# alphacep/vosk-tts

Hardware: AMD Instinct MI355X
Metric: audio_samples_per_sec (higher is better)
Workload: dtype f32

## Files before the change

vosk_tts_amd/csrc/engine_stages.hip.h:

```cpp
#pragma once
struct PendingLN { const float* raw = nullptr; const float* g = nullptr; const float* b = nullptr; const float* stat = nullptr; int nmb = 0; };

static bool enc_fold_ok(vits_session* s, const EncoderW& E, int B, int T) {
  if (E.layers.empty() || !s->xb || !s->y1b) return false;
  const EncLayerW& L = E.layers[0];
  return conv_takes_ln_prologue(conv_params(L.qkv, s->x, s->qkv, B, T, 1, 0)) &&
         conv_takes_ln_prologue(conv_params(L.f1, s->x, s->ffh, B, T, 1, (E.K - 1) / 2));
}

static void run_encoder(vits_session* s, const EncoderW& E, float* x, const int* len, int B, int T, int cond_layer,
                        int cond_off, const float* final_base, float* final_out, PendingLN* pend = nullptr) {
  vits_model* m = s->m;
  const int H = E.H, K = E.K;
  const int n = (int)E.layers.size();
  const bool fold = enc_fold_ok(s, E, B, T);
  bool pstat = fold && g_ln_stats && s->lnst && H % 16 == 0 && H / 16 <= 16;
  if (pstat) {
    const EncLayerW& L0 = E.layers[0];
    ConvParams Pp = conv_params(L0.f2, s->ffh, s->y1, B, T, 1, (K - 1) / 2);
    Pp.in_mask = 1; Pp.out_mask = 1; Pp.len = len;
    pstat = conv_writes_ln_stats(conv_params(L0.o, s->att, s->y1, B, T, 1, 0)) && conv_writes_ln_stats(Pp);
  }
  PendingLN prev;
  for (int i = 0; i < n; ++i) {
// ... 287 lines not shown
    ConvParams P;
    if (mono) {
      const MonoW& Mo = m->mono[f];
      const bool post_res = hp.flow_type == 5;
      hipLaunchKernelGGL(mono_x0_kernel, dim3(cdiv(Ty, 256), half, B), dim3(256), 0, s->stream, u, s->x, s->fh, s->len_y, I, half, Ty,
                         post_res ? 0.5f : 1.0f);
      run_encoder(s, Mo.enc, s->x, s->len_y, B, Ty, -1, -1, post_res ? nullptr : s->fh, s->fskip);
      {
        ProfScope ps(s, "flow.mono_couple", 2.0 * B * half * half * Ty, "mono_couple_kernel");
        launch_mono_couple_on(s->stream, s->fskip, u, Mo.post_w, Mo.post_b, s->len_y, v, B, half, Ty, post_res ? 1 : 0);
      }
      float* t = u; u = v; v = t;
    }
    if (hp.flow_type == 1) {
      hipLaunchKernelGGL(flow_x0_kernel, dim3(cdiv(Ty, 256), half, B), dim3(256), 0, s->stream, u, s->x, s->fh, s->len_y, I, half, Ty);
      run_encoder(s, C.enc, s->x, s->len_y, B, Ty, -1, -1, s->fh, s->fskip);
      P = conv_params(C.pre, s->fskip, s->fx, B, Ty, 1, 0);
      P.out_mask = 1; P.len = s->len_y;
      mark_masked(s, P, s->len_y);
      launch_conv(s, P, EPI_STORE, "flow.pre");
    } else {
      P = conv_params(C.pre, u, hp.flow_type == 0 ? s->fh : s->fx, B, Ty, 1, 0);
      P.x_ch_off = I - 1; P.x_ch_sign = -1; P.x_bstride = (long long)I * Ty;
      P.out_mask = 1; P.len = s->len_y;
      mark_masked(s, P, s->len_y);
      if (hp.flow_type == 0) P.g[0].y2 = s->x;
      launch_conv(s, P, EPI_STORE, "flow.pre");
      if (hp.flow_type == 0) run_encoder(s, C.enc, s->x, s->len_y, B, Ty, -1, -1, s->fh, s->fx);
    }
    const bool fold = g_wn_fold && !C.rsx.empty() && C.skip_post.w;
    const long long acts_b = (long long)(fold ? L : 1) * H * Ty;
    for (int i = 0; i < L; ++i) {
      float* acts = s->facts + (fold ? (size_t)i * H * Ty : 0);
      P = conv_params(C.in_layers[i], s->fx, acts, B, Ty, 1, (K5 - 1) / 2);
      P.Cout = H; P.H = H; P.y_bstride = acts_b;
      if (m->use_g) { P.bias_b = s->condv; P.bias_b_stride = m->cond_rows; P.bias_b_off = C.cond_off + i * 2 * H; }
      P.in_mask = 1; P.len = s->len_y;
      mark_masked(s, P, s->len_y);
      launch_conv(s, P, EPI_GATE, "flow.wn_in");
      if (fold) {
        if (i == L - 1) break;
        P = conv_params(C.rsx[i], acts, s->fx, B, Ty, 1, 0);
        P.x_bstride = acts_b;
        P.g[0].res = s->fx; P.out_mask = 1; P.len = s->len_y;
        mark_masked(s, P, s->len_y);
        launch_conv(s, P, EPI_STORE, "flow.wn_rs");
        continue;
      }
      P = conv_params(C.rs_layers[i], s->facts, nullptr, B, Ty, 1, 0);
      P.io = s->fx; P.skip = s->fskip; P.H = H; P.first = i == 0; P.last = i == L - 1; P.len = s->len_y;
      P.y_bstride = (long long)H * Ty;
      mark_masked(s, P, s->len_y);
      launch_conv(s, P, EPI_RESSKIP, "flow.wn_rs");
    }
    P = fold ? conv_params(C.skip_post, s->facts, nullptr, B, Ty, 1, 0) : conv_params(C.post, s->fskip, nullptr, B, Ty, 1, 0);
    P.u = u; P.io = v; P.H = half; P.len = s->len_y; P.y_bstride = (long long)I * Ty;
    mark_masked(s, P, s->len_y);
    launch_conv(s, P, EPI_COUPLE, "flow.post");
    float* t = u; u = v; v = t;
  }
  return u;
}

#define VITS_RAGGED_HALO 32
static void set_rag(ConvParams& P, const int* rag, int in_mul, int in_add, int out_mul, int out_add) {
  P.rag = rag; P.rag_in_mul = in_mul; P.rag_in_add = in_add; P.rag_out_mul = out_mul; P.rag_out_add = out_add; P.rag_out_cap_add = 0; P.rag_tab_add = 0;
}
static ConvParams dec_sum_conv(const ConvW& W, const float* const in[3], float in_scale, float slope, float* y, int B, int Cin, int Cout,
                               int Tin, int Tout, int pad_l, int taps, const UpW* U = nullptr, bool reflect = false) {
  ConvParams P = conv_params(W, in[0], y, B, Tin, 1, pad_l);
  P.g[0].x2 = in[1]; P.g[0].x3 = in[2]; P.g[0].K = taps;
  P.Cin = Cin; P.x_bstride = (long long)Cin * Tin;
  P.Cout = Cout; P.Tout = Tout; P.Tout_stride = U ? Tout * U->u : Tout; P.y_bstride = (long long)(U ? U->cout : Cout) * P.Tout_stride;
  P.in_slope = slope; P.in_scale = in_scale; P.reflect = reflect;
  if (U) {
    P.ups_u = U->u; P.ups_cout = U->cout;
    for (int r = 0; r < U->u; ++r) P.ups_shift[r] = U->shift[r];
  }
  return P;
}
static void run_decoder(vits_session* s, const float* z, bool mask_in, int B, int Ty, float* d_audio, long long audio_bstride,
                        bool ragged = false, bool cont = true) {
  vits_model* m = s->m;
  const vits_hparams& hp = m->hp;
  const DecGeom& G = m->geom;
  vits_session::DecBufs& W = s->dec;
  static const DecNeeds alone;
  const DecNeeds& ND = cont ? G.needs : alone;
  const int* rag = nullptr;
  const int* rag_tail = nullptr;
  if (ragged && (B > 1 || s->rag_b1)) {
    hipLaunchKernelGGL(ragged_len_kernel, dim3(cdiv(B + 1, 64)), dim3(64), 0, s->stream, s->len_y, s->len_rag, s->len_tail, B, Ty,
                       0, G.final_rate, ND.tail_cols);
    rag = s->len_rag;
    rag_tail = s->len_tail;
  }
  ConvParams P = conv_params(m->conv_pre, z, W.pre, B, Ty, 1, 3);
  if (mask_in) { P.in_mask = 1; P.len = s->len_y; }
  if (m->cond_dec_off >= 0) { P.bias_b = s->condv; P.bias_b_stride = m->cond_rows; P.bias_b_off = m->cond_dec_off; }
  set_rag(P, rag, 1, 0, 1, ND.pre_out);
  launch_conv(s, P, EPI_STORE, "dec.conv_pre");
  int prod_add = ND.pre_out;
  const float* in[3] = {W.pre, nullptr, nullptr};
  float in_scale = 1.f;
  const int nk = hp.n_resk;
  auto group = [](ConvGroup& g, const ConvW& w, const float* x, float* y, const float* res, int K, int dil) {
    g.x = x; g.w = w.w; g.wb = w.wb; g.bias = w.bias; g.y = y; g.res = res;
    g.K = K; g.dil = dil; g.pad_l = (K - 1) * dil / 2; g.n_sg = w.n_sg;
  };
  for (int i = 0; i < G.n_ups; ++i) {
    const DecGeom::Stage& S = G.st[i];
    const UpW& U = m->ups[i];
    const int p = i & 1, Ti = Ty * S.rate_in, T = Ty * S.rate_out;
    float* y = W.ups[p];
    float* const* xt = W.xt[p];
    float* const* x = W.x[p];
    P = dec_sum_conv(U.w, in, in_scale, 0.1f, y, B, S.cin, U.w.M, Ti, Ti, U.pad_l, U.taps, &U);
    set_rag(P, rag, S.rate_in, prod_add, S.rate_in, ND.ups_q[i]);
    launch_conv(s, P, EPI_STORE, "dec.ups", U.halo);
    prod_add = ND.ups_q[i] * S.u;
    for (int d = 0; d < hp.n_resd; ++d) {
      const ResBlockW* R = &m->rb[(size_t)i * nk];
      P = conv_params(R[0].c1[d], nullptr, nullptr, B, T, 1, 0);
      P.n_groups = nk; P.in_slope = 0.1f;
      for (int j = 0; j < nk; ++j) group(P.g[j], R[j].c1[d], d == 0 ? y : x[j], xt[j], nullptr, R[j].K, R[j].dil[d]);
      set_rag(P, rag, S.rate_out, prod_add, S.rate_out, ND.c1_out[i][d]);
      P.rag_tab_add = ND.c1_out[i][0];
      launch_conv(s, P, EPI_STORE, "dec.res_c1");
      for (int j = 0; j < nk; ++j) group(P.g[j], R[j].c2[d], xt[j], x[j], d == 0 ? y : x[j], R[j].K, 1);
      set_rag(P, rag, S.rate_out, ND.c1_out[i][d], S.rate_out, ND.c2_out[i][d]);
      P.rag_tab_add = ND.c1_out[i][0];
      launch_conv(s, P, EPI_STORE, "dec.res_c2");
      prod_add = ND.c2_out[i][d];
    }
    in[0] = x[0]; in[1] = nk > 1 ? x[1] : nullptr; in[2] = nk > 2 ? x[2] : nullptr;
    in_scale = 1.0f / (float)nk;
  }
  const int T = Ty * G.final_rate, Tp = T + G.reflect, C = G.st[G.n_ups - 1].cout;
  float* post = W.post;
  P = dec_sum_conv(m->conv_post, in, in_scale, 0.01f, post, B, C, G.post_rows, T, Tp, G.post_pad, 7, nullptr, G.reflect);
  set_rag(P, rag, G.final_rate, prod_add, G.final_rate, cont ? ND.post_out : (int)G.reflect);
  P.rag_out_cap_add = G.reflect;
  launch_conv(s, P, EPI_STORE, "dec.conv_post");
  if (!G.reflect) {
    hipLaunchKernelGGL(tanh_copy_kernel, dim3(cdiv(T, 256), B), dim3(256), 0, s->stream, post, d_audio, T, (long long)T, audio_bstride, rag_tail, 1);
    return;
  }
  float* mb = W.mb;
  const int S = hp.subbands, N = hp.istft_n_fft, hop = hp.istft_hop, Tm = T * hop;
  if (!G.has_mb) {
    if (g_tail_impl == 0) {
      ProfScope ps(s, "istft", 0, "istft_tail_kernel<false>");
      TailParams tp{post, m->istft_basis, nullptr, nullptr, d_audio, 1, N, hop, Tp, Tm, 0, audio_bstride, rag_tail, hop};
      hipLaunchKernelGGL(istft_tail_kernel<false>, dim3(cdiv(Tm, TAIL_SB), B), dim3(256), m->tail_lds, s->stream, tp);
    } else {
      ProfScope ps(s, "istft", 0, "istft_kernel");
      hipLaunchKernelGGL(istft_kernel, dim3(cdiv(Tm, 256), 1, B), dim3(256), 0, s->stream, post, m->istft_basis, d_audio, 1, N, hop, Tp, Tm,
                         audio_bstride, rag_tail, hop, 1);
    }
  } else if (g_tail_impl == 0) {
    ProfScope ps(s, "istft_pqmf", 0, "istft_tail_kernel<true>");
    TailParams tp{post, m->istft_basis, m->pqmf, mb, d_audio, S, N, hop, Tp, Tm, hp.pqmf_taps, audio_bstride, rag_tail, hop};
    hipLaunchKernelGGL(istft_tail_kernel<true>, dim3(cdiv(Tm, TAIL_MB), B), dim3(256), m->tail_lds, s->stream, tp);
  } else {
    {
      ProfScope ps(s, "istft", 0, "istft_kernel");
      hipLaunchKernelGGL(istft_kernel, dim3(cdiv(Tm, 256), S, B), dim3(256), 0, s->stream, post, m->istft_basis, mb, S, N, hop, Tp, Tm,
                         (long long)S * Tm, rag_tail, hop, 0);
    }
    {
      ProfScope ps(s, "pqmf", 0, "pqmf_synthesis_kernel");
      hipLaunchKernelGGL(pqmf_synthesis_kernel, dim3(cdiv(Tm * S, 256), B), dim3(256), 0, s->stream, mb, m->pqmf, d_audio, S,
                         hp.pqmf_taps, Tm, audio_bstride, rag_tail, hop * S);
    }
  }
}

struct HostStage {
  vits_model* m; vits_session* s = nullptr; std::vector<void*> tmp;
  PersistScope pscope;
  explicit HostStage(vits_model* m_) : m(m_), pscope(m_ ? m_->device : -1) {}
  ~HostStage() {
    if (s) {
      hipStreamSynchronize(s->stream);
      if (!tmp.empty()) {
        size_t want = s->stage_used + (s->stage_used >> 2) + (1 << 20);
        if (s->stage) hipFree(s->stage);
        s->stage = nullptr; s->stage_bytes = 0;
        void* p = nullptr;
        if (hipMalloc(&p, want) == hipSuccess) { s->stage = static_cast<char*>(p); s->stage_bytes = want; }
      }
      s->stage_used = 0;
      pool_release(m, s);
    }
    for (void* p : tmp) hipFree(p);
  }
  void* raw_alloc(size_t bytes) {
    bytes = align_up(bytes ? bytes : 1, 256);
    const size_t off = s->stage_used;
    s->stage_used += bytes;
    if (off + bytes <= s->stage_bytes) return s->stage + off;
    void* d = nullptr;
    if (hipMalloc(&d, bytes) != hipSuccess) return nullptr;
    tmp.push_back(d);
    return d;
  }
  template <typename T> T* to_dev(const T* h, size_t n) {
    if (!h) return nullptr;
    void* d = raw_alloc(n * sizeof(T));
    if (!d) return nullptr;
    hipMemcpyAsync(d, h, n * sizeof(T), hipMemcpyHostToDevice, s->stream);
    return static_cast<T*>(d);
  }
  template <typename T> T* dev_alloc(size_t n) { return static_cast<T*>(raw_alloc(n * sizeof(T))); }
};

static int begin_stage(HostStage& hs, int B, int Tx, int Ty, int roles = 7) {
  hipError_t e = hipSetDevice(hs.m->device);
  if (e != hipSuccess) return fail(VITS_ERR_DEVICE, "hipSetDevice failed: %s", hipGetErrorString(e));
  TRY(pool_acquire(hs.m, &hs.s));
  hs.s->ps_roles = roles;
  TRY(session_reserve(hs.s, B, Tx, Ty));
  return VITS_OK;
}

static void set_lengths(vits_session* s, const int64_t* d_len64, int* d_len32, int B, int clamp) {
  hipLaunchKernelGGL(lengths_to_i32_kernel, dim3(cdiv(B, 64)), dim3(64), 0, s->stream, d_len64, d_len32, B, clamp);
}


static void forward_device(vits_session* s, const int64_t* d_ids, const int64_t* d_len, int B, int Tx, const float* scales,
                           const int64_t* d_sid, const int32_t* d_forced, int Ty, uint64_t seed, float* d_audio, int64_t cap) {
  s->ragged = B > 1;
  s->tile_keys.clear();
  run_cond(s, d_sid, B, d_len, s->len_x, Tx);
  const bool with_sdp = !d_forced || s->sdp_always;
  float* z;
  if (persist_mask() == (PERSIST_SDP | PERSIST_ENC | PERSIST_FLOW) && B == 1 && Tx == s->Tx && Ty == s->Ty && s->ps_full[with_sdp].ok) {
    persist_launch(s, s->ps_full[with_sdp], "acoustic.persist", nullptr, scales[2], seed, d_ids, d_forced, scales[1], scales[0]);
    s->ea_pending = false;
    z = s->zB;
  } else {
    run_text_encoder(s, d_ids, B, Tx);
    if (with_sdp) run_duration(s, s->x, nullptr, scales[2], seed, B, Tx, true);
    run_durations(s, d_forced, scales[1], B, Tx, Ty);
    run_expand(s, nullptr, Ty, scales[0], seed, s->zA, B, Tx, Ty);
    z = run_flow(s, B, Ty);
  }
  run_decoder(s, z, true, B, Ty, d_audio, cap, true);
  s->ragged = false;
}
```

vosk_tts_amd/csrc/kernels_misc.hip.h:

```cpp
#pragma once
#include <hip/hip_runtime.h>
#include <stdint.h>

#define PI_F 3.14159265358979323846f

__host__ __device__ inline void philox4x32_10(uint32_t c[4], uint32_t k0, uint32_t k1) {
  for (int r = 0; r < 10; ++r) {
    uint64_t p0 = (uint64_t)0xD2511F53u * c[0], p1 = (uint64_t)0xCD9E8D57u * c[2];
    uint32_t n0 = (uint32_t)(p1 >> 32) ^ c[1] ^ k0, n1 = (uint32_t)p1;
    uint32_t n2 = (uint32_t)(p0 >> 32) ^ c[3] ^ k1, n3 = (uint32_t)p0;
    c[0] = n0; c[1] = n1; c[2] = n2; c[3] = n3;
    k0 += 0x9E3779B9u; k1 += 0xBB67AE85u;
  }
}
__device__ inline float philox_normal(uint64_t seed, uint32_t stream, uint32_t row, uint32_t t) {
  uint32_t c[4] = {t, row, stream, 0};
  philox4x32_10(c, (uint32_t)seed, (uint32_t)(seed >> 32));
  float u1 = ((float)c[0] + 0.5f) * (1.0f / 4294967296.0f);
  float u2 = ((float)c[1] + 0.5f) * (1.0f / 4294967296.0f);
  if (u1 < 1e-12f) u1 = 1e-12f;
  return sqrtf(-2.0f * logf(u1)) * cosf(6.28318530717958647692f * u2);
}

struct SynthDev {
// ... 771 lines not shown
    int d = 0;
    if (t < L) {
      if (forced) d = forced[(long long)b * T + t];
      else {
        const float lw = ea_z ? (ea_z[((long long)b * 2 + ea_row) * T + t] - ea_mu) * ea_sc : logw[(long long)b * T + t];
        d = (int)ceilf(expf(lw) * length_scale);
      }
    }
    if (d < 0) d = 0;
    dur[(long long)b * T + t] = d;
    s += d;
  }
  part[tid] = s;
  __syncthreads();
  if (tid == 0) {
    int run = 0;
    for (int i = 0; i < 256; ++i) { int v = part[i]; part[i] = run; run += v; }
    int yl = run < 1 ? 1 : run;
    if (Tcap > 0 && yl > Tcap) { atomicOr(err, 4); yl = Tcap; }
    ylen32[b] = yl;
    if (ylen64) ylen64[b] = yl;
  }
  __syncthreads();
  int run = part[tid];
  for (int t = t0; t < t0 + per && t < T; ++t) {
    run += dur[(long long)b * T + t];
    cum[(long long)b * T + t] = run;
  }
}

#define EXPAND_CPB 16
__global__ void __launch_bounds__(256) expand_prior_kernel(const float* stats, const int* cum, const int* ylen, const float* noise,
                                                           long long noise_stride, float noise_scale, uint64_t seed, float* z_p,
                                                           int I, int Tx, int Ty, int solo, const SynthDev* dv,
                                                           const unsigned long long* item_seeds) {
  const int f = blockIdx.x * 64 + (threadIdx.x & 63), cl = threadIdx.x >> 6, b = blockIdx.z;
  if (f >= Ty) return;
  if (dv) { noise_scale = dv->scales[0]; seed = dv->seed; }
  const int* cb = cum + (long long)b * Tx;
  int tok = -1;
  if (f < ylen[b] && f < cb[Tx - 1]) {
    int lo = 0, hi = Tx - 1;
    while (lo < hi) { int mid = (lo + hi) >> 1; if (cb[mid] > f) hi = mid; else lo = mid + 1; }
    tok = lo;
  }
  const int tk = tok >= 0 ? tok : 0;
#pragma unroll
  for (int i = 0; i < EXPAND_CPB / 4; ++i) {
    const int c = blockIdx.y * EXPAND_CPB + i * 4 + cl;
    if (c >= I) break;
    const float mu_ = stats[((long long)b * 2 * I + c) * Tx + tk];
    const float ls_ = stats[((long long)b * 2 * I + I + c) * Tx + tk];
    const float mu = tok >= 0 ? mu_ : 0.f, ls = tok >= 0 ? ls_ : 0.f;
    const float e = noise ? noise[((long long)b * I + c) * noise_stride + f]
                          : (solo ? philox_normal(item_seeds ? item_seeds[b] : seed + (uint64_t)b, 2, (uint32_t)c, (uint32_t)f)
                                  : philox_normal(seed, 2, (uint32_t)(b * I + c), (uint32_t)f));
    z_p[((long long)b * I + c) * Ty + f] = mu + e * expf(ls) * noise_scale;
  }
}

__global__ void ragged_tiles_kernel(const int* len, int B, int mul, int add, int cap, int tile, int* tile_start, int has_cap, int cap_add) {
  if (threadIdx.x != 0 || blockIdx.x != 0) return;
  int run = 0;
  if (has_cap) { const int c = len[B] * mul + cap_add; cap = c < cap ? c : cap; }
  for (int b = 0; b < B; ++b) {
    tile_start[b] = run;
    int cols = len[b] * mul + add;
    cols = cols < cap ? cols : cap;
    cols = cols < 0 ? 0 : cols;
    run += (cols + tile - 1) / tile;
  }
  tile_start[B] = run;
}

__global__ void ragged_len_kernel(const int* len_y, int* rag, int* tail, int B, int Ty, int halo, int tail_mul, int tail_add) {
  const int b = blockIdx.x * blockDim.x + threadIdx.x;
  if (b > B) return;
  int mx = 0;
  for (int i = 0; i < B; ++i) mx = len_y[i] > mx ? len_y[i] : mx;
  const int end = mx < Ty ? mx : Ty;
  if (b == B) { rag[B] = end; return; }
  const int v = len_y[b] + halo;
  rag[b] = v < end ? v : end;
  const int t = len_y[b] * tail_mul + tail_add, tc = end * tail_mul;
  tail[b] = t < tc ? t : tc;
}

__global__ void pcm16_kernel(const float* audio, long long a_bstride, int16_t* out, long long o_bstride, long long n, float scale,
                             const SynthDev* dv) {
  const long long i = (long long)blockIdx.x * blockDim.x + threadIdx.x;
  const int b = blockIdx.y;
  if (i >= n) return;
  if (dv) scale = dv->pcm_scale;
  float v = audio[(long long)b * a_bstride + i] * scale;
  v = v * 32767.0f;
  v = fminf(fmaxf(v, -32767.0f), 32767.0f);
  out[(long long)b * o_bstride + i] = (int16_t)(int)v;
}

__global__ void istft_kernel(const float* post, const float* basis, float* mb, int S, int N, int hop, int Tp, int Tm,
                             long long mb_bstride, const int* rag, int rag_mul, int zero_pad) {
  const int n = blockIdx.x * blockDim.x + threadIdx.x, s = blockIdx.y, b = blockIdx.z;
  if (n >= Tm) return;
  if (rag && n >= rag[b] * rag_mul) {
    if (zero_pad) mb[(long long)b * mb_bstride + (long long)s * Tm + n] = 0.f;
    return;
  }
  const int cut = N / 2 + 1, C = S * (N + 2);
  const int np = n + N / 2;
  int t_hi = np / hop;
  if (t_hi > Tp - 1) t_hi = Tp - 1;
  if (rag) {
    const int lim = rag[b] * rag_mul / hop;
    if (t_hi > lim) t_hi = lim;
  }
  int t_lo = (np - N + hop) / hop;
  if (np - N + 1 <= 0) t_lo = 0;
  const float* pb = post + ((long long)b * C + (long long)s * (N + 2)) * Tp;
  float a = 0.f;
  for (int t = t_lo; t <= t_hi; ++t) {
    const int j = np - t * hop;
    for (int k = 0; k < cut; ++k) {
      const float mag = expf(pb[(long long)k * Tp + t]);
      const float ph = PI_F * sinf(pb[(long long)(cut + k) * Tp + t]);
      float sn, cs;
      sincosf(ph, &sn, &cs);
      a += mag * cs * basis[k * N + j] + mag * sn * basis[(cut + k) * N + j];
    }
  }
  mb[(long long)b * mb_bstride + (long long)s * Tm + n] = a * ((float)N / (float)hop);
}

__global__ void pqmf_synthesis_kernel(const float* mb, const float* filt, float* audio, int S, int taps, int Tm,
                                      long long audio_bstride, const int* rag, int rag_mul) {
  const int t = blockIdx.x * blockDim.x + threadIdx.x, b = blockIdx.y;
  const int To = Tm * S, L = taps + 1, padl = taps / 2;
  if (t >= To) return;
  if (rag && t >= rag[b] * rag_mul) { audio[(long long)b * audio_bstride + t] = 0.f; return; }
  const int j0 = ((padl - t) % S + S) % S;
  const int u_lim = rag ? (rag[b] * rag_mul < To ? rag[b] * rag_mul : To) : To;
  float a = 0.f;
  for (int s = 0; s < S; ++s) {
    const float* xb = mb + ((long long)b * S + s) * Tm;
    for (int j = j0; j < L; j += S) {
      const int u = t + j - padl;
      if (u >= 0 && u < u_lim) a += filt[s * L + j] * (xb[u / S] * (float)S);
    }
  }
  audio[(long long)b * audio_bstride + t] = a;
}

#define TAIL_MB 64
#define TAIL_SB 256
struct TailParams {
  const float* post; const float* basis; const float* filt; float* mb; float* audio;
  int S, N, hop, Tp, Tm, taps;
  long long audio_bstride;
  const int* rag; int rag_mul;
};
__host__ __device__ inline size_t tail_lds_bytes(bool synth, int S, int N, int hop, int taps) {
  const int HM = synth ? (taps / 2 + S - 1) / S + 1 : 0, nsub = (synth ? TAIL_MB : TAIL_SB) + 2 * HM, FR = (nsub + N) / hop + 2;
  return ((size_t)2 * S * (N / 2 + 1) * FR + (synth ? (size_t)S * nsub : 0) + (size_t)(N + 2) * N + (synth ? (size_t)S * (taps + 1) : 0)) *
         sizeof(float);
}
template <bool kSynth>
__global__ void __launch_bounds__(256) istft_tail_kernel(const TailParams P) {
  extern __shared__ float sm[];
  kernarg_warm<sizeof(TailParams)>();
  constexpr int MB = kSynth ? TAIL_MB : TAIL_SB;
  const int tid = threadIdx.x, b = blockIdx.y, m0 = blockIdx.x * MB;
  const int S = kSynth ? P.S : 1, N = P.N, hop = P.hop, Tp = P.Tp, Tm = P.Tm;
  const int cut = N / 2 + 1, C = S * (N + 2), L = P.taps + 1, padl = P.taps / 2;
  const int HM = kSynth ? (padl + S - 1) / S + 1 : 0;
  const int n_lo = m0 - HM, nsub = MB + 2 * HM;
  const int FR = (nsub + N) / hop + 2;
  const int n_valid = P.rag ? (P.rag[b] * P.rag_mul < Tm ? P.rag[b] * P.rag_mul : Tm) : Tm;
  int f_hi_lim = Tp - 1;
  if (P.rag) { const int lim = P.rag[b] * P.rag_mul / hop; f_hi_lim = lim < f_hi_lim ? lim : f_hi_lim; }
  int f_lo = n_lo + N / 2 - N + 1;
  f_lo = f_lo <= 0 ? 0 : (f_lo + hop - 1) / hop;
  int f_hi = (n_lo + nsub - 1 + N / 2) / hop;
  f_hi = f_hi < f_hi_lim ? f_hi : f_hi_lim;
  const int nfr = f_hi - f_lo + 1;
  float* re = sm;
  float* im = re + S * cut * FR;
  float* sub = im + S * cut * FR;
  float* bas = sub + (kSynth ? S * nsub : 0);
  float* flt = bas + (N + 2) * N;
  for (int i = tid; i < (N + 2) * N; i += 256) bas[i] = P.basis[i];
  if (kSynth)
    for (int i = tid; i < S * L; i += 256) flt[i] = P.filt[i];
  for (int i = tid; i < S * cut * nfr; i += 256) {
    const int fr = i % nfr, sk = i / nfr, s = sk / cut, k = sk - s * cut;
    const float* pb = P.post + ((long long)b * C + (long long)s * (N + 2)) * Tp + f_lo + fr;
    const float mag = expf(pb[(long long)k * Tp]);
    const float ph = PI_F * sinf(pb[(long long)(cut + k) * Tp]);
    float sn, cs;
    sincosf(ph, &sn, &cs);
    re[sk * FR + fr] = mag * cs;
    im[sk * FR + fr] = mag * sn;
  }
  __syncthreads();
  for (int i = tid; i < S * nsub; i += 256) {
    const int s = i / nsub, q = i - s * nsub, n = n_lo + q;
    float a = 0.f;
    if (n >= 0 && n < n_valid) {
      const int np = n + N / 2;
      int t_hi = np / hop;
      t_hi = t_hi < f_hi_lim ? t_hi : f_hi_lim;
      int t_lo = (np - N + hop) / hop;
      if (np - N + 1 <= 0) t_lo = 0;
      for (int t = t_lo; t <= t_hi; ++t) {
        const int j = np - t * hop;
        const float* rp = re + (s * cut) * FR + (t - f_lo);
        const float* ip = im + (s * cut) * FR + (t - f_lo);
        for (int k = 0; k < cut; ++k) a += rp[k * FR] * bas[k * N + j] + ip[k * FR] * bas[(cut + k) * N + j];
      }
      a *= (float)N / (float)hop;
      if (kSynth && P.mb && q >= HM && q < HM + TAIL_MB) P.mb[((long long)b * S + s) * Tm + n] = a;
    }
    if (kSynth) sub[i] = a;
    else if (n < Tm) P.audio[(long long)b * P.audio_bstride + n] = a;
  }
  if (!kSynth) return;
  __syncthreads();
  const int To = Tm * S;
  for (int r = 0; r * 256 < TAIL_MB * S; ++r) {
    const int o = r * 256 + tid;
    const int t = m0 * S + o;
    if (o >= TAIL_MB * S || t >= To) continue;
    float a = 0.f;
    if (t < n_valid * S) {
      const int j0 = ((padl - t) % S + S) % S;
      for (int s = 0; s < S; ++s) {
        const float* xb = sub + s * nsub - n_lo;
        for (int j = j0; j < L; j += S) {
          const int u = t + j - padl;
          const int m = u >= 0 ? u / S : -((-u) / S);
          a += flt[s * L + j] * (xb[m] * (float)S);
        }
      }
    }
    P.audio[(long long)b * P.audio_bstride + t] = a;
  }
}

__global__ void tanh_copy_kernel(const float* x, float* y, int T, long long x_bstride, long long y_bstride, const int* rag, int rag_mul) {
  const int t = blockIdx.x * blockDim.x + threadIdx.x, b = blockIdx.y;
  if (t >= T) return;
  const bool live = !rag || t < rag[b] * rag_mul;
  y[(long long)b * y_bstride + t] = live ? tanhf(x[(long long)b * x_bstride + t]) : 0.f;
}

__global__ void window_copy_kernel(const float* __restrict__ z, long long zstride, int start, int W, float* __restrict__ dst) {
  const int t = blockIdx.x * blockDim.x + threadIdx.x, c = blockIdx.y;
  if (t < W) dst[(size_t)c * W + t] = z[(size_t)c * zstride + start + t];
}

struct WindowStarts { int v[8]; };
__global__ void window_copy_batch_kernel(const float* __restrict__ z, long long zstride, WindowStarts starts, int W, int I, float* __restrict__ dst) {
  const int t = blockIdx.x * blockDim.x + threadIdx.x, c = blockIdx.y, b = blockIdx.z;
  if (t < W) dst[((size_t)b * I + c) * W + t] = z[(size_t)c * zstride + starts.v[b] + t];
}

__global__ void __launch_bounds__(256) mas_kernel(const float* __restrict__ values, const int* __restrict__ t_ys,
                                                  const int* __restrict__ t_xs, int Ty, int Tx, unsigned char* __restrict__ diag,
                                                  int* __restrict__ paths) {
  extern __shared__ float rows[];
  const int b = blockIdx.x, tid = threadIdx.x, nt = blockDim.x;
  const int t_y = t_ys[b], t_x = t_xs[b];
  const float* v = values + (size_t)b * Ty * Tx;
  unsigned char* dg = diag + (size_t)b * Ty * Tx;
  int* path = paths + (size_t)b * Ty * Tx;
  for (size_t i = tid; i < (size_t)Ty * Tx; i += nt) path[i] = 0;
  if (t_y <= 0 || t_x <= 0) return;
  const float max_neg_val = -1e9f;
  for (int y = 0; y < t_y; ++y) {
    const float* prev = rows + ((y + 1) & 1) * Tx;
    float* cur = rows + (y & 1) * Tx;
    const int x0 = t_x + y - t_y > 0 ? t_x + y - t_y : 0, x1 = t_x < y + 1 ? t_x : y + 1;
    for (int x = x0 + tid; x < x1; x += nt) {
      const float v_cur = x == y ? max_neg_val : prev[x];
      const float v_prev = x == 0 ? (y == 0 ? 0.f : max_neg_val) : prev[x - 1];
      cur[x] = v[(size_t)y * Tx + x] + (v_prev > v_cur ? v_prev : v_cur);
      dg[(size_t)y * Tx + x] = (x != 0 && x != y && v_cur < v_prev) ? 1 : 0;
    }
    __syncthreads();
  }
  __threadfence_block();
  if (tid == 0) {
    int index = t_x - 1;
    for (int y = t_y - 1; y >= 0; --y) {
      path[(size_t)y * Tx + index] = 1;
      if (index != 0 && (index == y || dg[(size_t)y * Tx + index])) index -= 1;
    }
  }
}


__global__ void stts_embed_kernel(const int64_t* ids, const float* emb, const float* pemb, float* x, int H, int E, int Pd, int T,
                                  int n_vocab, float es, float ps, int* err) {
  const int t = blockIdx.x * blockDim.x + threadIdx.x, c = blockIdx.y, b = blockIdx.z;
  if (t >= T) return;
  const int s = c < E ? 0 : 1 + (c - E) / Pd;
  long long id = ids[((long long)b * 5 + s) * T + t];
  if (id < 0 || id >= n_vocab) { atomicOr(err, 1); id = 0; }
  x[((long long)b * H + c) * T + t] = c < E ? emb[id * E + c] * es : pemb[id * Pd + (c - E) % Pd] * ps;
}
__global__ void mask_rows_kernel(float* x, const int* len, int C, int T) {
  const int t = blockIdx.x * blockDim.x + threadIdx.x, c = blockIdx.y, b = blockIdx.z;
  if (t < T && t >= len[b]) x[((long long)b * C + c) * T + t] = 0.f;
}
__global__ void rope_kernel(float* qkv, int H, int T, int heads, int dk) {
  const int d = dk / 2, d2 = d / 2;
  const int t = blockIdx.x * blockDim.x + threadIdx.x, hj = blockIdx.y, b = blockIdx.z >> 1, which = blockIdx.z & 1;
  if (t >= T) return;
  const int h = hj / d2, j = hj % d2;
  const float theta = 1.0f / powf(10000.0f, (float)(2 * j) / (float)d);
  const float ang = (float)t * theta, cs = cosf(ang), sn = sinf(ang);
  float* r0 = qkv + (((long long)b * 3 + which) * H + h * dk + j) * T + t;
  float* r1 = r0 + (long long)d2 * T;
  const float x0 = *r0, x1 = *r1;
  *r0 = x0 * cs - x1 * sn;
  *r1 = x1 * cs + x0 * sn;
}
__global__ void film_mask_kernel(const float* h, float* out, const float* film, const int* len, int H, int T) {
  const int t = blockIdx.x * blockDim.x + threadIdx.x, c = blockIdx.y, b = blockIdx.z;
  if (t >= T) return;
  const long long o = ((long long)b * H + c) * T + t;
  out[o] = t < len[b] ? film[c] * h[o] + film[H + c] : 0.f;
}
__global__ void gemv_rows_kernel(const float* W, const float* bias, const float* x, int x_stride, float* y, int y_stride, int rows,
                                 int cols, int act) {
  const int lane = threadIdx.x & 63, row = blockIdx.x * (blockDim.x >> 6) + (threadIdx.x >> 6), n = blockIdx.y;
  if (row >= rows) return;
  float a = 0.f;
  for (int j = lane; j < cols; j += 64) a += W[(long long)row * cols + j] * x[(long long)n * x_stride + j];
  for (int o = 32; o > 0; o >>= 1) a += __shfl_down(a, o, 64);
  if (lane == 0) {
    a += bias ? bias[row] : 0.f;
    y[(long long)n * y_stride + row] = act == 1 ? a / (1.0f + __expf(-a)) : a;
  }
}
__global__ void copy_rows_kernel(const float* src, long long sb, float* dst, long long db, int T) {
  const int t = blockIdx.x * blockDim.x + threadIdx.x, r = blockIdx.y, b = blockIdx.z;
  if (t < T) dst[(long long)b * db + (long long)r * T + t] = src[(long long)b * sb + (long long)r * T + t];
}
struct SttsDev { float temperature; float pad; unsigned long long seed; };
__global__ void cfm_init_kernel(float* cat, long long cat_b, const float* noise, long long nstride, float temperature, uint64_t seed,
                                int NF, int T, int B, int cfg, const SttsDev* dv, const unsigned long long* item_seeds = nullptr) {
  const int t = blockIdx.x * blockDim.x + threadIdx.x, c = blockIdx.y, b = blockIdx.z;
  if (t >= T) return;
  if (dv) { temperature = dv->temperature; seed = dv->seed; }
  const float v = (noise ? noise[(long long)c * nstride + t]
                         : philox_normal(item_seeds ? item_seeds[b] : seed + (uint64_t)b, 3u, (uint32_t)c, (uint32_t)t)) * temperature;
  cat[(long long)b * cat_b + (long long)c * T + t] = v;
  if (cfg) cat[(long long)(B + b) * cat_b + (long long)c * T + t] = v;
}
__global__ void cfm_euler_kernel(float* cat, long long cat_b, const float* d, float dt, float g, int NF, int T, int B, int cfg) {
  const int t = blockIdx.x * blockDim.x + threadIdx.x, c = blockIdx.y, b = blockIdx.z;
  if (t >= T) return;
  const long long o = (long long)c * T + t;
  float d0 = d[(long long)b * NF * T + o];
  if (cfg) d0 = d0 + g * (d0 - d[(long long)(B + b) * NF * T + o]);
  const float x = cat[(long long)b * cat_b + o] + dt * d0;
  cat[(long long)b * cat_b + o] = x;
  if (cfg) cat[(long long)(B + b) * cat_b + o] = x;
}
__global__ void stts_expand_kernel(const float* x, const int* cum, int Tx, float* mu_y, int CC, int T, const float* pde, float* pau) {
  const int t = blockIdx.x * blockDim.x + threadIdx.x, c = blockIdx.y, b = blockIdx.z;
  if (t >= T) return;
  cum += (long long)b * Tx;
  int lo = 0, hi = Tx;
  while (lo < hi) { const int mid = (lo + hi) >> 1; if (cum[mid] > t) hi = mid; else lo = mid + 1; }
  const bool valid = lo < Tx;
  mu_y[((long long)b * CC + c) * T + t] = valid ? x[((long long)b * CC + c) * Tx + lo] : 0.f;
  if (c == 0) pau[(long long)b * T + t] = (valid && pde) ? pde[(long long)b * Tx + lo] : 0.f;
}
__global__ void stts_mel_kernel(const float* cat, long long cat_b, int T, const float* pau, float* mel, int NF, int Tm, const int* len,
                                float mel_std, float mel_mean) {
  const int t = blockIdx.x * blockDim.x + threadIdx.x, c = blockIdx.y, b = blockIdx.z;
  if (t >= Tm) return;
  const float* cb = cat + (long long)b * cat_b;
  float v = 0.f;
  if (t < len[b]) v = (pau[(long long)b * T + t] > 0.f ? cb[(long long)c * T] : cb[(long long)c * T + t]) * mel_std + mel_mean;
  mel[((long long)b * NF + c) * Tm + t] = v;
}
__global__ void gather_rows_kernel(float* dst, const float* table, const int64_t* idx, int G, int n_rows, int* err) {
  const int j = blockIdx.x * blockDim.x + threadIdx.x, b = blockIdx.y;
  if (j >= G) return;
  long long r = idx[b];
  if (r < 0 || r >= n_rows) { if (j == 0) atomicOr(err, 2); r = 0; }
  dst[(long long)b * G + j] = table[r * G + j];
// ... 552 lines not shown
```

Baseline: 45.10 million.

## Restructure iSTFT tail kernel with interleaved LDS layout, 512 threads, unrolled inner loops

Rewrites the fused iSTFT/PQMF tail kernel. The real and imaginary spectra and the basis are stored interleaved as float2 in LDS, and the block grows from 256 to 512 threads. Global loads in phase one are batched four per thread ahead of the transcendental math, and the frame and PQMF tap loops are unrolled with strength-reduced indexing and no per-iteration divisions. The goal is fewer LDS instructions and less index arithmetic. The cost is more registers per thread and a basis copy that assumes alignment, and the reordered arithmetic may change results slightly.

New measurement: 45.53 million (median of 6 runs). Within noise of the previous version (+1.0%).

```diff
diff --git a/vosk_tts_amd/csrc/engine_stages.hip.h b/vosk_tts_amd/csrc/engine_stages.hip.h
--- a/vosk_tts_amd/csrc/engine_stages.hip.h
+++ b/vosk_tts_amd/csrc/engine_stages.hip.h
@@ -463,7 +463,7 @@
     if (g_tail_impl == 0) {
       ProfScope ps(s, "istft", 0, "istft_tail_kernel<false>");
       TailParams tp{post, m->istft_basis, nullptr, nullptr, d_audio, 1, N, hop, Tp, Tm, 0, audio_bstride, rag_tail, hop};
-      hipLaunchKernelGGL(istft_tail_kernel<false>, dim3(cdiv(Tm, TAIL_SB), B), dim3(256), m->tail_lds, s->stream, tp);
+      hipLaunchKernelGGL(istft_tail_kernel<false>, dim3(cdiv(Tm, TAIL_SB), B), dim3(TAIL_THREADS), m->tail_lds, s->stream, tp);
     } else {
       ProfScope ps(s, "istft", 0, "istft_kernel");
       hipLaunchKernelGGL(istft_kernel, dim3(cdiv(Tm, 256), 1, B), dim3(256), 0, s->stream, post, m->istft_basis, d_audio, 1, N, hop, Tp, Tm,
@@ -472,7 +472,7 @@
   } else if (g_tail_impl == 0) {
     ProfScope ps(s, "istft_pqmf", 0, "istft_tail_kernel<true>");
     TailParams tp{post, m->istft_basis, m->pqmf, mb, d_audio, S, N, hop, Tp, Tm, hp.pqmf_taps, audio_bstride, rag_tail, hop};
-    hipLaunchKernelGGL(istft_tail_kernel<true>, dim3(cdiv(Tm, TAIL_MB), B), dim3(256), m->tail_lds, s->stream, tp);
+    hipLaunchKernelGGL(istft_tail_kernel<true>, dim3(cdiv(Tm, TAIL_MB), B), dim3(TAIL_THREADS), m->tail_lds, s->stream, tp);
   } else {
     {
       ProfScope ps(s, "istft", 0, "istft_kernel");
diff --git a/vosk_tts_amd/csrc/kernels_misc.hip.h b/vosk_tts_amd/csrc/kernels_misc.hip.h
--- a/vosk_tts_amd/csrc/kernels_misc.hip.h
+++ b/vosk_tts_amd/csrc/kernels_misc.hip.h
@@ -947,6 +947,7 @@
 
 #define TAIL_MB 64
 #define TAIL_SB 256
+#define TAIL_THREADS 512
 struct TailParams {
   const float* post; const float* basis; const float* filt; float* mb; float* audio;
   int S, N, hop, Tp, Tm, taps;
@@ -958,11 +959,42 @@
   return ((size_t)2 * S * (N / 2 + 1) * FR + (synth ? (size_t)S * nsub : 0) + (size_t)(N + 2) * N + (synth ? (size_t)S * (taps + 1) : 0)) *
          sizeof(float);
 }
+template <int K>
+__device__ __forceinline__ float tail_terms(float a, const float2* x, const float2* w, int FR, int N) {
+#pragma clang fp contract(off)
+  float2 xv[K], wv[K];
+#pragma unroll
+  for (int k = 0; k < K; ++k) xv[k] = x[k * FR], wv[k] = w[k * N];
+#pragma unroll
+  for (int k = 0; k < K; ++k) a += xv[k].x * wv[k].x + xv[k].y * wv[k].y;
+  return a;
+}
+__device__ __forceinline__ float tail_frame_sum(float a, const float2* x, const float2* w, int cut, int FR, int N) {
+  for (int g = cut >> 3; g > 0; --g, x += 8 * FR, w += 8 * N) a = tail_terms<8>(a, x, w, FR, N);
+  if (cut & 4) { a = tail_terms<4>(a, x, w, FR, N); x += 4 * FR, w += 4 * N; }
+  if (cut & 2) { a = tail_terms<2>(a, x, w, FR, N); x += 2 * FR, w += 2 * N; }
+  if (cut & 1) a = tail_terms<1>(a, x, w, FR, N);
+  return a;
+}
+__device__ __forceinline__ float tail_sample_sum(const float2* x, const float2* w, int nt, int hop, int cut, int FR, int N) {
+  float a = 0.f;
+  for (int r = 0; r < nt; ++r, ++x, w -= hop) a = tail_frame_sum(a, x, w, cut, FR, N);
+  return a;
+}
+template <int K>
+__device__ __forceinline__ float tail_taps(float a, const float* f, const float* x, int S, float fS) {
+  float fv[K], xv[K];
+#pragma unroll
+  for (int i = 0; i < K; ++i) fv[i] = f[i * S], xv[i] = x[i];
+#pragma unroll
+  for (int i = 0; i < K; ++i) a = __builtin_fmaf(fv[i], xv[i] * fS, a);
+  return a;
+}
 template <bool kSynth>
-__global__ void __launch_bounds__(256) istft_tail_kernel(const TailParams P) {
+__global__ void __launch_bounds__(TAIL_THREADS) istft_tail_kernel(const TailParams P) {
   extern __shared__ float sm[];
   kernarg_warm<sizeof(TailParams)>();
-  constexpr int MB = kSynth ? TAIL_MB : TAIL_SB;
+  constexpr int MB = kSynth ? TAIL_MB : TAIL_SB, NT = TAIL_THREADS, U = 4;
   const int tid = threadIdx.x, b = blockIdx.y, m0 = blockIdx.x * MB;
   const int S = kSynth ? P.S : 1, N = P.N, hop = P.hop, Tp = P.Tp, Tm = P.Tm;
   const int cut = N / 2 + 1, C = S * (N + 2), L = P.taps + 1, padl = P.taps / 2;
@@ -977,63 +1009,128 @@
   int f_hi = (n_lo + nsub - 1 + N / 2) / hop;
   f_hi = f_hi < f_hi_lim ? f_hi : f_hi_lim;
   const int nfr = f_hi - f_lo + 1;
-  float* re = sm;
-  float* im = re + S * cut * FR;
-  float* sub = im + S * cut * FR;
-  float* bas = sub + (kSynth ? S * nsub : 0);
-  float* flt = bas + (N + 2) * N;
-  for (int i = tid; i < (N + 2) * N; i += 256) bas[i] = P.basis[i];
-  if (kSynth)
-    for (int i = tid; i < S * L; i += 256) flt[i] = P.filt[i];
-  for (int i = tid; i < S * cut * nfr; i += 256) {
-    const int fr = i % nfr, sk = i / nfr, s = sk / cut, k = sk - s * cut;
-    const float* pb = P.post + ((long long)b * C + (long long)s * (N + 2)) * Tp + f_lo + fr;
-    const float mag = expf(pb[(long long)k * Tp]);
-    const float ph = PI_F * sinf(pb[(long long)(cut + k) * Tp]);
-    float sn, cs;
-    sincosf(ph, &sn, &cs);
-    re[sk * FR + fr] = mag * cs;
-    im[sk * FR + fr] = mag * sn;
-  }
-  __syncthreads();
-  for (int i = tid; i < S * nsub; i += 256) {
-    const int s = i / nsub, q = i - s * nsub, n = n_lo + q;
-    float a = 0.f;
-    if (n >= 0 && n < n_valid) {
-      const int np = n + N / 2;
-      int t_hi = np / hop;
-      t_hi = t_hi < f_hi_lim ? t_hi : f_hi_lim;
-      int t_lo = (np - N + hop) / hop;
-      if (np - N + 1 <= 0) t_lo = 0;
-      for (int t = t_lo; t <= t_hi; ++t) {
-        const int j = np - t * hop;
-        const float* rp = re + (s * cut) * FR + (t - f_lo);
-        const float* ip = im + (s * cut) * FR + (t - f_lo);
-        for (int k = 0; k < cut; ++k) a += rp[k * FR] * bas[k * N + j] + ip[k * FR] * bas[(cut + k) * N + j];
+  float2* bas = reinterpret_cast<float2*>(sm);
+  float2* ri = bas + cut * N;
+  float* sub = reinterpret_cast<float*>(ri + S * cut * FR);
+  float* flt = sub + (kSynth ? S * nsub : 0);
+
+  const int total = S * cut * nfr, nfd = nfr > 0 ? nfr : 1;
+  const int dsk = NT / nfd, dfr = NT - dsk * nfd, dsc = dsk / cut, dk = dsk - dsc * cut;
+  const long long cutTp = (long long)cut * Tp, wrapTp = (long long)(N + 2 - cut) * Tp;
+  const long long doff = (long long)(dsc * (N + 2) + dk) * Tp + dfr;
+  const int didx = dsk * FR + dfr;
+  const float* pb = P.post + (long long)b * C * Tp + f_lo;
+  int it = tid, fr, k, idx;
+  long long off;
+  {
+    const int sk = tid / nfd, s = sk / cut;
+    fr = tid - sk * nfd, k = sk - s * cut, idx = sk * FR + fr;
+    off = (long long)(s * (N + 2) + k) * Tp + fr;
+  }
+  float xm[U], xp[U];
+  int ix[U];
+  auto p1_load = [&]() {
+#pragma unroll
+    for (int u = 0; u < U; ++u) {
+      const bool on = it < total;
+      ix[u] = on ? idx : -1;
+      xm[u] = on ? pb[off] : 0.f;
+      xp[u] = on ? pb[off + cutTp] : 0.f;
+      it += NT, fr += dfr, k += dk, off += doff, idx += didx;
+      if (fr >= nfr) fr -= nfr, ++k, off += Tp - nfr, idx += FR - nfr;
+      if (k >= cut) k -= cut, off += wrapTp;
+    }
+  };
+  p1_load();
+  {
+    const int cn = cut * N;
+    if ((N & 3) == 0) {
+      const float4* g = reinterpret_cast<const float4*>(P.basis);
+      float4* d = reinterpret_cast<float4*>(sm);
+      for (int u = tid; u < cn / 4; u += NT) {
+        const float4 re4 = g[u], im4 = g[u + cn / 4];
+        d[2 * u] = make_float4(re4.x, im4.x, re4.y, im4.y);
+        d[2 * u + 1] = make_float4(re4.z, im4.z, re4.w, im4.w);
       }
-      a *= (float)N / (float)hop;
-      if (kSynth && P.mb && q >= HM && q < HM + TAIL_MB) P.mb[((long long)b * S + s) * Tm + n] = a;
-    }
-    if (kSynth) sub[i] = a;
-    else if (n < Tm) P.audio[(long long)b * P.audio_bstride + n] = a;
+    } else {
+      for (int e = tid; e < cn; e += NT) bas[e] = make_float2(P.basis[e], P.basis[e + cn]);
+    }
+    if (kSynth) {
+      const int nf = S * L;
+      const float4* g = reinterpret_cast<const float4*>(P.filt);
+      for (int u = tid; u < nf / 4; u += NT) {
+        const float4 v = g[u];
+        flt[4 * u] = v.x, flt[4 * u + 1] = v.y, flt[4 * u + 2] = v.z, flt[4 * u + 3] = v.w;
+      }
+      for (int e = (nf & ~3) + tid; e < nf; e += NT) flt[e] = P.filt[e];
+    }
+  }
+  for (int g = U * NT;; g += U * NT) {
+#pragma unroll
+    for (int u = 0; u < U; ++u) {
+      if (ix[u] < 0) continue;
+      const float mag = expf(xm[u]);
+      const float ph = PI_F * sinf(xp[u]);
+      float sn, cs;
+      sincosf(ph, &sn, &cs);
+      ri[ix[u]] = make_float2(mag * cs, mag * sn);
+    }
+    if (g >= total) break;
+    p1_load();
+  }
+  __syncthreads();
+
+  {
+    const float gain = (float)N / (float)hop;
+    const int R = N / hop, ds2 = NT / nsub, dq = NT - ds2 * nsub;
+    int s = tid / nsub, q = tid - s * nsub;
+    for (int i = tid; i < S * nsub; i += NT) {
+      const int n = n_lo + q, np = n + N / 2;
+      const bool live = n >= 0 && n < n_valid;
+      const int th = np / hop;
+      const int t_hi = th < f_hi_lim ? th : f_hi_lim;
+      const int t_lo = np - N + 1 <= 0 ? 0 : th - (R - 1);
+      const float2* x = ri + (s * cut) * FR + (t_lo - f_lo);
+      const float2* w = bas + (np - t_lo * hop);
+      float a = 0.f;
+      if (__all(!live || t_hi - t_lo + 1 == R)) {
+        if (live) a = tail_sample_sum(x, w, R, hop, cut, FR, N);
+      } else if (live) {
+        a = tail_sample_sum(x, w, t_hi - t_lo + 1, hop, cut, FR, N);
+      }
+      if (live) {
+        a *= gain;
+        if (kSynth && P.mb && q >= HM && q < HM + TAIL_MB) P.mb[((long long)b * S + s) * Tm + n] = a;
+      }
+      if (kSynth) sub[i] = a;
+      else if (n < Tm) P.audio[(long long)b * P.audio_bstride + n] = a;
+      q += dq, s += ds2;
+      if (q >= nsub) q -= nsub, ++s;
+    }
   }
   if (!kSynth) return;
   __syncthreads();
-  const int To = Tm * S;
-  for (int r = 0; r * 256 < TAIL_MB * S; ++r) {
-    const int o = r * 256 + tid;
+
+  const int To = Tm * S, nt = L / S, rem = L - nt * S;
+  const float fS = (float)S;
+  for (int o = tid; o < TAIL_MB * S; o += NT) {
     const int t = m0 * S + o;
-    if (o >= TAIL_MB * S || t >= To) continue;
+    if (t >= To) break;
     float a = 0.f;
     if (t < n_valid * S) {
-      const int j0 = ((padl - t) % S + S) % S;
-      for (int s = 0; s < S; ++s) {
-        const float* xb = sub + s * nsub - n_lo;
-        for (int j = j0; j < L; j += S) {
-          const int u = t + j - padl;
-          const int m = u >= 0 ? u / S : -((-u) / S);
-          a += flt[s * L + j] * (xb[m] * (float)S);
-        }
+      const int v = t - padl + S * HM;
+      const int vq = v / S, rr = v - vq * S, j0 = rr ? S - rr : 0;
+      const float* xb = sub + (vq - HM + (rr != 0) - n_lo);
+      const float* fb = flt + j0;
+      const bool more = j0 < rem;
+      for (int s = 0; s < S; ++s, xb += nsub, fb += L) {
+        const float* f = fb;
+        const float* x = xb;
+        for (int g = nt >> 3; g > 0; --g, f += 8 * S, x += 8) a = tail_taps<8>(a, f, x, S, fS);
+        if (nt & 4) { a = tail_taps<4>(a, f, x, S, fS); f += 4 * S, x += 4; }
+        if (nt & 2) { a = tail_taps<2>(a, f, x, S, fS); f += 2 * S, x += 2; }
+        if (nt & 1) { a = tail_taps<1>(a, f, x, S, fS); f += S, x += 1; }
+        if (more) a = tail_taps<1>(a, f, x, S, fS);
       }
     }
     P.audio[(long long)b * P.audio_bstride + t] = a;
```
